# CarminLiu/ORB_SLAM2_aruco

Hardware: AMD Instinct MI355X
Metric: frames/s (ORB+ArUco extract+match, 640x480 mono) (higher is better)
Workload: dtype u8

## Files before the change

### orb_slam2_aruco_amd/csrc/match_kernels.hip

```cpp
#include <climits>

#include "host_stage.hpp"
#include "orbfe_common.hpp"
#include "wave_dpp.hpp"

namespace orbfe {

__device__ __forceinline__ int hamming256(const uint4& a0, const uint4& a1, const uint4& b0, const uint4& b1)
{
    int d = __popc(a0.x ^ b0.x);
    d += __popc(a0.y ^ b0.y);
    d += __popc(a0.z ^ b0.z);
    d += __popc(a0.w ^ b0.w);
    d += __popc(a1.x ^ b1.x);
    d += __popc(a1.y ^ b1.y);
    d += __popc(a1.z ^ b1.z);
    d += __popc(a1.w ^ b1.w);
    return d;
}

#define KNN_TILE 256

__global__ __launch_bounds__(256) void k_knn2_tiles(const uint8_t* __restrict__ Q, const int32_t* __restrict__ nq_arr,
                                                    size_t q_stride, int max_nq, const uint8_t* __restrict__ T,
                                                    const int32_t* __restrict__ nt_arr, size_t t_stride, int chunk,
                                                    int init, int32_t* __restrict__ best_idx,
                                                    int32_t* __restrict__ best_dist, int32_t* __restrict__ second_dist)
{
    __shared__ uint4 st[KNN_TILE * 2];
    const int pair = blockIdx.y, split = blockIdx.z, nsplit = gridDim.z;
    const int nq = nq_arr ? nq_arr[pair] : max_nq;
    const int nt = nt_arr[pair];
    const int q = blockIdx.x * 256 + threadIdx.x;
    if (blockIdx.x * 256 >= nq) return;
    const uint4* Qp = reinterpret_cast<const uint4*>(Q + (size_t)pair * q_stride);
    const uint4* Tp = reinterpret_cast<const uint4*>(T + (size_t)pair * t_stride);
    uint4 a0 = make_uint4(0, 0, 0, 0), a1 = a0;
    if (q < nq) { a0 = Qp[2 * q]; a1 = Qp[2 * q + 1]; }
    int best = init, second = init, idx = -1;
    const int t_begin = split * chunk, t_end = min(nt, t_begin + chunk);
    for (int t0 = t_begin; t0 < t_end; t0 += KNN_TILE) {
        const int m = min(KNN_TILE, t_end - t0);
        __syncthreads();
        for (int i = threadIdx.x; i < 2 * m; i += 256) st[i] = Tp[2 * t0 + i];
        __syncthreads();
        for (int t = 0; t < m; t++) {
            const int d = hamming256(a0, a1, st[2 * t], st[2 * t + 1]);
            if (d < best) { second = best; best = d; idx = t0 + t; }
            else if (d < second) second = d;
        }
    }
    if (q < nq) {
        const size_t o = ((size_t)pair * nsplit + split) * max_nq + q;
        best_idx[o] = idx; best_dist[o] = best; second_dist[o] = second;
    }
}

#define KM_WAVES 8
#define KM_CHUNK 128
#define KM_ROWB 272
typedef int v4i __attribute__((ext_vector_type(4)));
typedef int v16i __attribute__((ext_vector_type(16)));

__device__ __forceinline__ int med3i(int a, int b, int c) { return max(min(a, b), min(max(a, b), c)); }
__device__ __forceinline__ int spread4(uint32_t x) { return (int)(__umul24(x & 15u, 0x00204081u) & 0x01010101u); }
__device__ __forceinline__ int x255_1(int x)
{
    int t;
    asm("v_lshlrev_b32 %0, 8, %1" : "=v"(t) : "v"(x));
    return t - x;
}
__device__ __forceinline__ v4i x255(v4i p)
{
    v4i r;
    r.x = x255_1(p.x); r.y = x255_1(p.y); r.z = x255_1(p.z); r.w = x255_1(p.w);
    return r;
}
__device__ __forceinline__ v4i spread16(uint32_t bits)
{
    v4i r;
    r.x = spread4(bits); r.y = spread4(bits >> 4); r.z = spread4(bits >> 8); r.w = spread4(bits >> 12);
    return r;
}

__global__ __launch_bounds__(KM_WAVES * 64) __attribute__((amdgpu_waves_per_eu(4, 4))) void k_knn2_mfma(const uint8_t* __restrict__ Q, const int32_t* __restrict__ nq_arr,
                                                             size_t q_stride, int max_nq, const uint8_t* __restrict__ T,
                                                             const int32_t* __restrict__ nt_arr, size_t t_stride, int chunk,
                                                             int init, int32_t* __restrict__ best_idx,
                                                             int32_t* __restrict__ best_dist,
                                                             int32_t* __restrict__ second_dist)
{
    constexpr int KM_LDS = KM_CHUNK * KM_ROWB > KM_WAVES * 32 * 33 * 4 ? KM_CHUNK * KM_ROWB : KM_WAVES * 32 * 33 * 4;
    __shared__ __align__(16) unsigned char s_u[KM_LDS];
    unsigned char* s_t = s_u;
    int (*s_red)[32][33] = reinterpret_cast<int (*)[32][33]>(s_u);
    __shared__ int s_pt[KM_CHUNK];
    const int pair = blockIdx.y, tid = threadIdx.x, lane = tid & 63, wid = tid >> 6;
    const int nq = nq_arr ? nq_arr[pair] : max_nq;
    const int split = blockIdx.z, nsplit = gridDim.z;
    const int t_begin = split * chunk, nt = min(nt_arr[pair], t_begin + chunk);
    const int q0 = blockIdx.x * (KM_WAVES * 32);
    if (q0 >= nq) return;
    const uint32_t* Qp = reinterpret_cast<const uint32_t*>(Q + (size_t)pair * q_stride);
    const uint32_t* Tp = reinterpret_cast<const uint32_t*>(T + (size_t)pair * t_stride);
    const int col = lane & 31, half = lane >> 5;
    const int ie = min(init, 257);

    const int qa = q0 + 32 * wid + col;
    v4i a[8];
    {
        const uint4* qrow = reinterpret_cast<const uint4*>(Qp) + (size_t)min(qa, nq - 1) * 2;
        const uint4 d0 = qrow[0], d1 = qrow[1];
        const uint32_t w[8] = {d0.x, d0.y, d0.z, d0.w, d1.x, d1.y, d1.z, d1.w};
#pragma unroll
        for (int s2 = 0; s2 < 8; s2++) {
            const v4i p = spread16((qa < nq ? w[s2] : 0u) >> (16 * half));
            a[s2] = x255(p);
        }
    }
    int bestk[16], secondk[16];
#pragma unroll
    for (int r = 0; r < 16; r++) bestk[r] = secondk[r] = 0x7fffffff;

    const int ctr = tid >> 2, cpart = tid & 3;
    const uint2* Tp2 = reinterpret_cast<const uint2*>(Tp);
    uint2 nxt = make_uint2(0u, 0u);
    if (t_begin < nt) nxt = Tp2[(size_t)min(t_begin + ctr, nt - 1) * 4 + cpart];
    for (int t0 = t_begin; t0 < nt; t0 += KM_CHUNK) {
        const int m = min(KM_CHUNK, nt - t0);
        uint2 w = nxt;
        if (ctr >= m) w = make_uint2(0u, 0u);
        __syncthreads();
        {
            v4i* dst = reinterpret_cast<v4i*>(s_t + ctr * KM_ROWB + cpart * 64);
            dst[0] = spread16(w.x);
            dst[1] = spread16(w.x >> 16);
            dst[2] = spread16(w.y);
            dst[3] = spread16(w.y >> 16);
            int pc = __popc(w.x) + __popc(w.y);
            pc += ORBFE_DPP(0, pc, 0xb1, 0xf);
            pc += ORBFE_DPP(0, pc, 0x4e, 0xf);
            if (cpart == 0) s_pt[ctr] = pc;
        }
        if (t0 + KM_CHUNK < nt) nxt = Tp2[(size_t)min(t0 + KM_CHUNK + ctr, nt - 1) * 4 + cpart];
        __syncthreads();
#pragma unroll
        for (int tt = 0; tt < KM_CHUNK; tt += 32) {
            v16i acc = {0, 0, 0, 0, 0, 0, 0, 0, 0, 0, 0, 0, 0, 0, 0, 0};
            const unsigned char* brow = s_t + (tt + col) * KM_ROWB + 16 * half;
            v4i b[8];
#pragma unroll
            for (int s2 = 0; s2 < 8; s2++) b[s2] = *reinterpret_cast<const v4i*>(brow + 32 * s2);
            const int pt = s_pt[tt + col];
#pragma unroll
            for (int s2 = 0; s2 < 8; s2++) acc = __builtin_amdgcn_mfma_i32_32x32x32_i8(a[s2], b[s2], acc, 0, 0, 0);
            const uint32_t cj = (tt + col < m) ? (((uint32_t)pt << 16) | (uint32_t)(t0 + tt + col)) : 0x7fffffffu;
#pragma unroll
            for (int r = 0; r < 16; r++) {
                const int key = (int)(((uint32_t)acc[r] << 17) + cj);
                secondk[r] = med3i(bestk[r], secondk[r], key);
                bestk[r] = min(bestk[r], key);
            }
        }
    }
    __syncthreads();
#pragma unroll
    for (int pass = 0; pass < 2; pass++) {
        __builtin_amdgcn_wave_barrier();
#pragma unroll
        for (int r = 0; r < 16; r++) s_red[wid][(r & 3) + 8 * (r >> 2) + 4 * half][col] = pass == 0 ? bestk[r] : secondk[r];
        __builtin_amdgcn_wave_barrier();
        int b1 = 0x7fffffff, b2 = 0x7fffffff;
#pragma unroll
        for (int c = 0; c < 16; c++) {
            const int key = s_red[wid][col][16 * half + c];
            b2 = med3i(b1, b2, key);
            b1 = min(b1, key);
        }
        const int o1 = __shfl_xor(b1, 32), o2 = __shfl_xor(b2, 32);
        const int n1 = min(b1, o1);
        const int n2 = min(max(b1, o1), min(b2, o2));
        if (pass == 0) { bestk[0] = n1; bestk[1] = n2; }
        else { secondk[0] = n1; }
    }
    if (half == 0) {
        const int qr = q0 + 32 * wid + col;
        if (qr < nq) {
            uint4 d0 = reinterpret_cast<const uint4*>(Qp)[(size_t)qr * 2], d1 = reinterpret_cast<const uint4*>(Qp)[(size_t)qr * 2 + 1];
            const int pq = __popc(d0.x) + __popc(d0.y) + __popc(d0.z) + __popc(d0.w) + __popc(d1.x) + __popc(d1.y) + __popc(d1.z) + __popc(d1.w);
            const int kb = bestk[0], ks = min(bestk[1], secondk[0]);
            int bd = (kb >> 16) + pq, sd = (ks >> 16) + pq, bi = kb & 0xffff;
            if (bd >= ie) { bd = init; bi = -1; }
            if (sd >= ie) sd = init;
            const size_t o = ((size_t)pair * nsplit + split) * max_nq + qr;
            best_idx[o] = bi; best_dist[o] = bd; second_dist[o] = sd;
        }
    }
}

__global__ void k_knn2_merge(const int32_t* __restrict__ pidx, const int32_t* __restrict__ pbest,
                             const int32_t* __restrict__ psecond, int nsplit, int max_nq,
                             const int32_t* __restrict__ nq_arr, int32_t* __restrict__ best_idx,
                             int32_t* __restrict__ best_dist, int32_t* __restrict__ second_dist)
{
    const int pair = blockIdx.y;
    const int q = blockIdx.x * blockDim.x + threadIdx.x;
    const int nq = nq_arr ? nq_arr[pair] : max_nq;
    if (q >= nq) return;
    int best = INT_MAX, second = INT_MAX, idx = -1;
    for (int s = 0; s < nsplit; s++) {
        const size_t o = ((size_t)pair * nsplit + s) * max_nq + q;
        const int b = pbest[o], sc = psecond[o], i = pidx[o];
        if (s == 0) { best = b; second = sc; idx = i; continue; }
        if (b < best) { second = min(best, sc); best = b; idx = i; }
        else second = min(second, b);
    }
    const size_t o = (size_t)pair * max_nq + q;
    best_idx[o] = idx; best_dist[o] = best; second_dist[o] = second;
}

#define GRID_COLS 64
#define GRID_ROWS 48


#define SFI_MAXL0 1024
struct SfiGrid {
    int32_t* nl0;
    int32_t* nq;
    uint32_t* sorted;
    float2* xy;
    float* ang;
    uint4* desc;
    uint16_t* query;
    float2* qxy;
    int32_t* cursor;
};
#define SFI_GRID_THREADS 256
#define SFI_CURSOR_PAD 64
#define SFI_ROWS_BX 64
#define SFI_POOL_LDS 6144
#define SFI_ROW_BITS 11

__global__ __launch_bounds__(SFI_GRID_THREADS) void k_sfi_grid(const orbfe_keypoint* __restrict__ kps, const uint8_t* __restrict__ desc,
                                                               const int32_t* __restrict__ nkp, int capacity, int nframes, float4 bnd,
                                                               SfiGrid G, int32_t* __restrict__ overflow)
{
    __shared__ __align__(16) uint32_t s_key[SFI_MAXL0 + 4];
    __shared__ int s_nl0;
    const int f = blockIdx.x, tid = threadIdx.x, lane = tid & 63, wid = tid >> 6;
    const orbfe_keypoint* k = kps + (size_t)f * capacity;
    const uint8_t* d = desc + (size_t)f * capacity * 32;
    const int n = nkp[f];
    const float mnMinX = bnd.x, mnMinY = bnd.y;
    const float invW = __fdiv_rn((float)GRID_COLS, bnd.z - bnd.x);
    const float invH = __fdiv_rn((float)GRID_ROWS, bnd.w - bnd.y);
    if (tid == 0) { s_nl0 = 0; if (f < nframes - 1) G.cursor[(size_t)f * SFI_CURSOR_PAD] = 0; }
    __syncthreads();
    for (int i = tid; i < n; i += SFI_GRID_THREADS) {
        const orbfe_keypoint kp = k[i];
        if (kp.octave != 0) continue;
        const int px = (int)roundf(__fmul_rn(kp.x - mnMinX, invW));
        const int py = (int)roundf(__fmul_rn(kp.y - mnMinY, invH));
        if (px >= 0 && px < GRID_COLS && py >= 0 && py < GRID_ROWS) {
            const int e = atomicAdd(&s_nl0, 1);
            if (e < SFI_MAXL0) s_key[e] = ((uint32_t)(px * GRID_ROWS + py) << 16) | (uint32_t)i;
        }
    }
    if (wid == 0) {
        int nq = 0;
        uint16_t* qo = G.query + (size_t)f * SFI_MAXL0;
        float2* qp = G.qxy + (size_t)f * SFI_MAXL0;
        for (int i0 = 0; i0 < n; i0 += 64) {
            const int i = i0 + lane;
            orbfe_keypoint kp;
            kp.octave = 1;
            if (i < n) kp = k[i];
            const bool isq = i < n && kp.octave <= 0;
            const unsigned long long m = __ballot(isq);
            const int pos = nq + __builtin_amdgcn_mbcnt_hi((unsigned)(m >> 32), __builtin_amdgcn_mbcnt_lo((unsigned)m, 0));
            if (isq && pos < SFI_MAXL0) { qo[pos] = (uint16_t)i; qp[pos] = make_float2(kp.x, kp.y); }
            nq += __popcll(m);
        }
        if (lane == 0) {
            if (nq > SFI_MAXL0) { atomicMax(overflow, nq); nq = SFI_MAXL0; }
            G.nq[f] = nq;
        }
    }
    __syncthreads();
    int nl0 = s_nl0;
    if (nl0 > SFI_MAXL0) { if (tid == 0) atomicMax(overflow, nl0); nl0 = SFI_MAXL0; }
    if (tid == 0) G.nl0[f] = nl0;
    if (tid < 4) s_key[nl0 + tid] = 0xffffffffu;
    __syncthreads();
    const uint4* k4 = reinterpret_cast<const uint4*>(s_key);
    for (int e = tid; e < nl0; e += SFI_GRID_THREADS) {
        const uint32_t key = s_key[e];
        int r = 0;
        for (int j = 0; j < (nl0 + 3) / 4; j++) {
            const uint4 v = k4[j];
            r += (v.x < key) + (v.y < key) + (v.z < key) + (v.w < key);
        }
        const int i2 = key & 0xffff;
        const orbfe_keypoint kp = k[i2];
        const size_t o = (size_t)f * SFI_MAXL0 + r;
        G.sorted[o] = key;
        G.xy[o] = make_float2(kp.x, kp.y);
        G.ang[o] = kp.angle;
        G.desc[2 * o] = reinterpret_cast<const uint4*>(d)[2 * i2];
        G.desc[2 * o + 1] = reinterpret_cast<const uint4*>(d)[2 * i2 + 1];
    }
}

struct SfiWindow { float x, y, r; int minx, maxx, miny, maxy; };
__device__ __forceinline__ int sfi_chunks4(const SfiGrid& G, size_t g2, int nl0, int c0, int lane, const SfiWindow& W, const uint4& a0,
                                           const uint4& a1, int base, int* keys)
{
    uint32_t cell[4];
    float2 xy[4];
#pragma unroll
    for (int k = 0; k < 4; k++) {
        const int j = (c0 + k) * 64 + lane;
        cell[k] = 0xffffffffu; xy[k] = make_float2(0.f, 0.f);
        if (j < nl0) { cell[k] = G.sorted[g2 + j] >> 16; xy[k] = G.xy[g2 + j]; }
    }
    bool ok[4];
    uint4 b0[4], b1[4];
#pragma unroll
    for (int k = 0; k < 4; k++) {
        const int cx = (int)(cell[k] / GRID_ROWS), cy = (int)(cell[k] - (uint32_t)cx * GRID_ROWS);
        ok[k] = cell[k] != 0xffffffffu && cx >= W.minx && cx <= W.maxx && cy >= W.miny && cy <= W.maxy && fabsf(xy[k].x - W.x) < W.r &&
                fabsf(xy[k].y - W.y) < W.r;
        if (ok[k]) { const size_t o = 2 * (g2 + (size_t)((c0 + k) * 64 + lane)); b0[k] = G.desc[o]; b1[k] = G.desc[o + 1]; }
    }
    int n = 0;
#pragma unroll
    for (int k = 0; k < 4; k++) {
        const unsigned long long m = __ballot(ok[k]);
        keys[k] = 0x7fffffff;
        if (ok[k]) {
            const int pos = base + n + __builtin_amdgcn_mbcnt_hi((unsigned)(m >> 32), __builtin_amdgcn_mbcnt_lo((unsigned)m, 0));
            const int dd = hamming256(a0, a1, b0[k], b1[k]);
            keys[k] = (min(dd, 255) << 20) | (pos << 10) | ((c0 + k) * 64 + lane);
        }
        n += (int)__popcll(m);
// ... 681 lines not shown
    int nlevels, strict_max, level_below, level_above;
    float log_scale, th;
    int use_T2;
    float T2[12];
    int frame_variant;
};

__global__ __launch_bounds__(256) void k_project_map_points(const float* __restrict__ p3Dw, const uint8_t* __restrict__ valid,
                                                            const float* __restrict__ min_dist, const float* __restrict__ max_dist,
                                                            const float* __restrict__ normal, int n, ProjectParams P,
                                                            SbpQuery* __restrict__ queries)
{
    const int i = blockIdx.x * 256 + threadIdx.x;
    if (i >= n) return;
    SbpQuery Q{0.0f, 0.0f, -1.0f, 0, 0};
    if (!valid || valid[i]) {
        const float X = p3Dw[3 * i], Y = p3Dw[3 * i + 1], Z = p3Dw[3 * i + 2];
        float xc = __fadd_rn(__fadd_rn(__fadd_rn(__fmul_rn(P.T[0], X), __fmul_rn(P.T[1], Y)), __fmul_rn(P.T[2], Z)), P.T[3]);
        float yc = __fadd_rn(__fadd_rn(__fadd_rn(__fmul_rn(P.T[4], X), __fmul_rn(P.T[5], Y)), __fmul_rn(P.T[6], Z)), P.T[7]);
        float zc = __fadd_rn(__fadd_rn(__fadd_rn(__fmul_rn(P.T[8], X), __fmul_rn(P.T[9], Y)), __fmul_rn(P.T[10], Z)), P.T[11]);
        if (P.use_T2) {
            const float a = xc, b = yc, c = zc;
            xc = __fadd_rn(__fadd_rn(__fadd_rn(__fmul_rn(P.T2[0], a), __fmul_rn(P.T2[1], b)), __fmul_rn(P.T2[2], c)), P.T2[3]);
            yc = __fadd_rn(__fadd_rn(__fadd_rn(__fmul_rn(P.T2[4], a), __fmul_rn(P.T2[5], b)), __fmul_rn(P.T2[6], c)), P.T2[7]);
            zc = __fadd_rn(__fadd_rn(__fadd_rn(__fmul_rn(P.T2[8], a), __fmul_rn(P.T2[9], b)), __fmul_rn(P.T2[10], c)), P.T2[11]);
        }
        float u = 0.0f, v = 0.0f;
        bool inside = false;
        if (P.frame_variant) {
            const float invzc = (float)(1.0 / (double)zc);
            u = __fadd_rn(__fmul_rn(__fmul_rn(P.K[0], xc), invzc), P.K[2]);
            v = __fadd_rn(__fmul_rn(__fmul_rn(P.K[1], yc), invzc), P.K[3]);
            inside = u >= P.bnd[0] && u <= P.bnd[2] && v >= P.bnd[1] && v <= P.bnd[3];
        } else if (!(zc < 0.0f)) {
            const float invz = __fdiv_rn(1.0f, zc);
            u = __fadd_rn(__fmul_rn(P.K[0], __fmul_rn(xc, invz)), P.K[2]);
            v = __fadd_rn(__fmul_rn(P.K[1], __fmul_rn(yc, invz)), P.K[3]);
            inside = P.strict_max ? (u >= P.bnd[0] && u < P.bnd[2] && v >= P.bnd[1] && v < P.bnd[3])
                                  : (u >= P.bnd[0] && u <= P.bnd[2] && v >= P.bnd[1] && v <= P.bnd[3]);
        }
        if (inside) {
            const float px = P.use_T2 ? xc : X - P.Ow[0], py = P.use_T2 ? yc : Y - P.Ow[1], pz = P.use_T2 ? zc : Z - P.Ow[2];
            const float dist3D = (float)sqrt((double)px * px + (double)py * py + (double)pz * pz);
            const float mfMax = max_dist[i];
            bool ok = !(dist3D < __fmul_rn(0.8f, min_dist[i]) || dist3D > __fmul_rn(1.2f, mfMax));
            if (ok && normal) {
                const double dot = (double)px * normal[3 * i] + (double)py * normal[3 * i + 1] + (double)pz * normal[3 * i + 2];
                ok = !(dot < 0.5 * (double)dist3D);
            }
            if (ok) {
                const float ratio = __fdiv_rn(mfMax, dist3D);
                int lvl = (int)ceilf(__fdiv_rn((float)log((double)ratio), P.log_scale));
                if (lvl < 0) lvl = 0;
                else if (lvl >= P.nlevels) lvl = P.nlevels - 1;
                Q = SbpQuery{u, v, __fmul_rn(P.th, P.scale[lvl]), lvl - P.level_below, lvl + P.level_above};
            }
        }
    }
    queries[i] = Q;
}

#define DD_MAXN 256
__global__ __launch_bounds__(256) void k_distinctive(const uint8_t* __restrict__ desc, const int32_t* __restrict__ offsets, int npoints,
                                                     int32_t* __restrict__ best_idx, uint8_t* __restrict__ best_desc)
{
    const int p = blockIdx.x * 4 + (threadIdx.x >> 6), lane = threadIdx.x & 63;
    if (p >= npoints) return;
    const int o0 = offsets[p], N = min(offsets[p + 1] - o0, DD_MAXN);
    if (N <= 0) {
        if (lane == 0) best_idx[p] = -1;
        return;
    }
    const uint4* D = reinterpret_cast<const uint4*>(desc) + (size_t)o0 * 2;
    uint32_t w[4][8];
#pragma unroll
    for (int c = 0; c < 4; c++) {
        const int j = lane + 64 * c;
        uint4 a = make_uint4(0, 0, 0, 0), b = a;
        if (j < N) { a = D[2 * j]; b = D[2 * j + 1]; }
        w[c][0] = a.x; w[c][1] = a.y; w[c][2] = a.z; w[c][3] = a.w; w[c][4] = b.x; w[c][5] = b.y; w[c][6] = b.z; w[c][7] = b.w;
    }
    const int k = (int)(0.5 * (double)(N - 1));
    int best_median = 0x7fffffff, best = 0;
    for (int i = 0; i < N; i++) {
        uint32_t r[8];
        const int src_lane = i & 63, src_c = i >> 6;
#pragma unroll
        for (int q = 0; q < 8; q++) {
            const uint32_t v = src_c == 0 ? w[0][q] : src_c == 1 ? w[1][q] : src_c == 2 ? w[2][q] : w[3][q];
            r[q] = (uint32_t)__builtin_amdgcn_readlane((int)v, src_lane);
        }
        int d[4];
#pragma unroll
        for (int c = 0; c < 4; c++) {
            int s_ = 0;
#pragma unroll
            for (int q = 0; q < 8; q++) s_ += __popc(w[c][q] ^ r[q]);
            d[c] = s_;
        }
        int lo = 0, hi = 256;
        while (lo < hi) {
            const int mid = (lo + hi) >> 1;
            int cnt = 0;
#pragma unroll
            for (int c = 0; c < 4; c++) cnt += __popcll(__ballot(lane + 64 * c < N && d[c] <= mid));
            if (cnt >= k + 1) hi = mid; else lo = mid + 1;
        }
        if (lo < best_median) { best_median = lo; best = i; }
    }
    if (lane == 0) best_idx[p] = best;
    if (best_desc && lane < 8) reinterpret_cast<uint32_t*>(best_desc)[(size_t)p * 8 + lane] = reinterpret_cast<const uint32_t*>(D)[(size_t)best * 8 + lane];
}

struct MatchWorkspace {
    DevBuf pidx, pbest, psecond, csr_cnt, csr_idx, csr_dist, scratch;
    DevBuf sbp_batch_overflow;
    DevBuf sfi_overflow;
    DevBuf q, obest;
    int csr_per_pair = 0;
    int sbp_stride = 0;
};
static thread_local ThreadWorkspaces<MatchWorkspace> tl_ws;
static MatchWorkspace& ws(hipStream_t s) { return tl_ws.get(s); }
static thread_local ThreadWorkspaces<HostStage> tl_stage;
HostStage& match_host_stage() { return tl_stage.get(); }
static int ensure_sticky_flag(DevBuf& b)
{
    if (b.p) return ORBFE_OK;
    int rc = b.ensure(16);
    if (rc) return rc;
    ORBFE_HIP(hipMemset(b.p, 0, 16));
    return ORBFE_OK;
}

static int g_knn2_path = 0;
#ifdef ORBFE_ABLATION
int g_orb_skip = 0, g_aruco_skip = 0;
#endif

static int knn2_launch(const uint8_t* d_Q, const int32_t* d_nq, size_t q_stride, int max_nq, const uint8_t* d_T,
                       const int32_t* d_nt, size_t t_stride, int max_nt, int npairs, int init, int32_t* d_best_idx,
                       int32_t* d_best_dist, int32_t* d_second_dist, hipStream_t s)
{
    const bool mfma_ok = max_nt <= 65535 && init > 0;
    const bool use_mfma = mfma_ok && g_knn2_path != 1;
    const int qtiles = (max_nq + 255) / 256;
    int nsplit = 1, chunk;
    const long long wgs = (long long)qtiles * npairs;
    if (use_mfma) {
        const int max_split = (max_nt + KM_CHUNK - 1) / KM_CHUNK;
        if (wgs < 512) nsplit = (int)std::max<long long>(1, std::min<long long>(512 / wgs, max_split));
        chunk = (max_nt + nsplit - 1) / nsplit;
        chunk = std::max(KM_CHUNK, (chunk + KM_CHUNK - 1) / KM_CHUNK * KM_CHUNK);
    } else {
        if (wgs < 1024) {
            nsplit = (int)std::min<long long>((1024 + wgs - 1) / wgs, (max_nt + KNN_TILE - 1) / KNN_TILE);
            if (nsplit < 1) nsplit = 1;
        }
        chunk = (max_nt + nsplit - 1) / nsplit;
        chunk = std::max(KNN_TILE, (chunk + KNN_TILE - 1) / KNN_TILE * KNN_TILE);
    }
    nsplit = std::max(1, (max_nt + chunk - 1) / chunk);
    const dim3 mgrid((max_nq + KM_WAVES * 32 - 1) / (KM_WAVES * 32), npairs, nsplit);
    if (nsplit == 1) {
        if (use_mfma)
            hipLaunchKernelGGL(k_knn2_mfma, mgrid, dim3(KM_WAVES * 64), 0, s, d_Q, d_nq, q_stride, max_nq, d_T, d_nt, t_stride, chunk, init,
                               d_best_idx, d_best_dist, d_second_dist);
        else
            hipLaunchKernelGGL(k_knn2_tiles, dim3(qtiles, npairs, 1), dim3(256), 0, s, d_Q, d_nq, q_stride, max_nq, d_T,
                               d_nt, t_stride, chunk, init, d_best_idx, d_best_dist, d_second_dist);
    } else {
        MatchWorkspace& w = ws(s);
        const size_t nb = (size_t)npairs * nsplit * max_nq * 4;
        int rc;
        if ((rc = w.pidx.ensure(nb)) || (rc = w.pbest.ensure(nb)) || (rc = w.psecond.ensure(nb))) return rc;
        if (use_mfma)
            hipLaunchKernelGGL(k_knn2_mfma, mgrid, dim3(KM_WAVES * 64), 0, s, d_Q, d_nq, q_stride, max_nq, d_T, d_nt, t_stride, chunk, init,
                               w.pidx.as<int32_t>(), w.pbest.as<int32_t>(), w.psecond.as<int32_t>());
        else
            hipLaunchKernelGGL(k_knn2_tiles, dim3(qtiles, npairs, nsplit), dim3(256), 0, s, d_Q, d_nq, q_stride, max_nq,
                               d_T, d_nt, t_stride, chunk, init, w.pidx.as<int32_t>(), w.pbest.as<int32_t>(),
                               w.psecond.as<int32_t>());
        hipLaunchKernelGGL(k_knn2_merge, dim3(qtiles, npairs), dim3(256), 0, s, w.pidx.as<int32_t>(),
                           w.pbest.as<int32_t>(), w.psecond.as<int32_t>(), nsplit, max_nq, d_nq, d_best_idx,
                           d_best_dist, d_second_dist);
    }
    ORBFE_HIP(hipGetLastError());
    return ORBFE_OK;
}

static float4 frame_bounds(int cols, int rows, const float* bounds)
{
    return bounds ? make_float4(bounds[0], bounds[1], bounds[2], bounds[3]) : make_float4(0.f, 0.f, (float)cols, (float)rows);
}

static int sfi_launch(const orbfe_keypoint* d_kps, const uint8_t* d_desc, const int32_t* d_n, int capacity, int npairs,
                      float4 bnd, int window, float nnratio, int check_ori, const float* d_prev_in,
                      float* d_prev_out, int32_t* d_m12, int32_t* d_nm, hipStream_t s, MatchWorkspace& w)
{
    if (capacity > 65535) return fail(ORBFE_ERR_INVALID, "capacity above 65535 keypoints per frame is unsupported");
    const int pool_cap = std::max((w.csr_per_pair + 3) / 4 * 4, 16384);
    w.csr_per_pair = pool_cap;
    const int nframes = npairs + 1;
    const size_t F = (size_t)nframes * SFI_MAXL0;
    int rc;
    if ((rc = w.csr_cnt.ensure((size_t)nframes * (2 + SFI_CURSOR_PAD) * 4 + 64)) || (rc = w.csr_idx.ensure(F * (4 + 8 + 4 + 32 + 8 + 2) + 256)) ||
        (rc = w.csr_dist.ensure((size_t)npairs * pool_cap * 4 + 512 )) || (rc = w.scratch.ensure((size_t)npairs * SFI_MAXL0 * 4)))
        return rc;
    if (!w.sfi_overflow.p) {
        if ((rc = w.sfi_overflow.ensure(16))) return rc;
        ORBFE_HIP(hipMemset(w.sfi_overflow.p, 0, 16));
    }
    SfiGrid G;
    G.nl0 = w.csr_cnt.as<int32_t>();
    G.nq = G.nl0 + nframes;
    G.cursor = G.nq + nframes;
    uint8_t* b = w.csr_idx.as<uint8_t>();
    G.desc = reinterpret_cast<uint4*>(b); b += F * 32;
    G.xy = reinterpret_cast<float2*>(b); b += F * 8;
    G.sorted = reinterpret_cast<uint32_t*>(b); b += F * 4;
    G.qxy = reinterpret_cast<float2*>(b); b += F * 8;
    G.ang = reinterpret_cast<float*>(b); b += F * 4;
    G.query = reinterpret_cast<uint16_t*>(b);
    int32_t* ovf = w.sfi_overflow.as<int32_t>();
    hipLaunchKernelGGL(k_sfi_grid, dim3(nframes), dim3(SFI_GRID_THREADS), 0, s, d_kps, d_desc, d_n, capacity, nframes, bnd, G, ovf);
    hipLaunchKernelGGL(k_sfi_rows, dim3(SFI_ROWS_BX, npairs), dim3(SFI_ROWS_WAVES * 64), 0, s, d_kps, d_desc, capacity, bnd, (float)window, d_prev_in, G,
                       w.csr_dist.as<uint32_t>(), pool_cap, w.scratch.as<uint32_t>(), ovf);
    hipLaunchKernelGGL(k_sfi_accept, dim3(npairs), dim3(64), 0, s, d_kps, d_n, capacity, nnratio, check_ori, d_prev_in, d_prev_out, d_m12,
                       d_nm, G, w.csr_dist.as<uint32_t>(), pool_cap, w.scratch.as<uint32_t>());
    ORBFE_HIP(hipGetLastError());
    return ORBFE_OK;
}

static int sfi_take_flags(MatchWorkspace& w, const int32_t* f, hipStream_t s, int32_t* need)
{
    if (f[0] || f[1]) ORBFE_HIP(hipMemsetAsync(w.sfi_overflow.p, 0, 8, s));
    if (f[1] > w.csr_per_pair) w.csr_per_pair = (f[1] + 1023) / 1024 * 1024;
    *need = f[0] > SFI_MAXL0 ? f[0] : f[1];
    if (f[0] > SFI_MAXL0) return fail(ORBFE_ERR_CAPACITY, "%d level-0 keypoints in a frame exceed the supported %d", f[0], SFI_MAXL0);
    return ORBFE_OK;
}

static void sbp_grow_stride(MatchWorkspace& w, int overflow)
{
    if (overflow > w.sbp_stride) w.sbp_stride = (overflow + 63) / 64 * 64;
}

static int sbp_launch(MatchWorkspace& w, SbpBatch B, int nframes, float4 bnd, int mode, int th_high, float nnratio, float factor,
                      int check_ori, hipStream_t s)
{
    if (B.capacity > 65535) return fail(ORBFE_ERR_INVALID, "more than 65535 keypoints per frame are unsupported");
    int ncap = 64;
    while (ncap < B.capacity) ncap <<= 1;
    const size_t lds = (size_t)ncap * (4 + 8 + 1 + 1) + (SBP_CELLS + 2) * 2 + 64;
    if (lds > 150 * 1024) return fail(ORBFE_ERR_CAPACITY, "%d keypoints do not fit the grid kernel's LDS", B.capacity);
    w.sbp_stride = std::max(w.sbp_stride, 128);
    const size_t NQ = (size_t)nframes * B.qcapacity;
    int rc;
    if ((rc = w.csr_idx.ensure(NQ * w.sbp_stride * 2)) || (rc = w.csr_dist.ensure(NQ * w.sbp_stride)) || (rc = w.csr_cnt.ensure(NQ * 4)) ||
        (rc = ensure_dyn_lds(reinterpret_cast<const void*>(&k_search_by_projection_batch), lds)))
        return rc;
    B.row_rank = w.csr_idx.as<uint16_t>(); B.row_dist = w.csr_dist.as<uint8_t>(); B.row_cnt = w.csr_cnt.as<int32_t>(); B.row_stride = w.sbp_stride;
    hipLaunchKernelGGL(k_search_by_projection_batch, dim3(nframes), dim3(SBP_THREADS), lds, s, B, ncap, bnd, mode, th_high, nnratio, factor,
                       check_ori);
    ORBFE_HIP(hipGetLastError());
    return ORBFE_OK;
}

struct SbpHostCall {
    const orbfe_keypoint* kps; const uint8_t* desc; int n; float4 bnd;
    const uint8_t* taken;
    int nq; const uint8_t* qdesc; const uint8_t* q_observed; const float* q_angle;
    const orbfe_window_query* window;
    const float* x3Dw; const uint8_t* valid;
    const orbfe_keypoint* kps_last; const float* Tcw; const float* K4; const float* scale; int nlevels; float th;
    const ProjectParams* P; const float* min_dist; const float* max_dist; const float* normal;
    int mode, th_high; float nnratio, factor; int check_ori;
    double chi2; const float* inv_sigma2;
    int32_t *best_idx, *best_dist, *best_level, *second_dist, *second_level, *match, *match_cur, *nmatches;
    uint8_t* taken_out;
};

static int sbp_host_run(const SbpHostCall& c)
{
    HostStage& w = match_host_stage();
    const size_t n = (size_t)c.n, nq = (size_t)c.nq, kb = sizeof(orbfe_keypoint);
    IoLayout l;
    const size_t s_kps = l.take(n * kb), s_desc = l.take(n * 32), s_q = l.take(nq * sizeof(SbpQuery)), s_qdesc = l.take(nq * 32);
    const size_t s_obs = l.take(nq), s_angle = l.take(nq * 4), s_x3 = l.take(nq * 12), s_valid = l.take(nq);
    const size_t s_last = l.take(c.kps_last ? nq * kb : 0), s_cam = l.take(c.kps_last ? (12 + 16) * 4 : 0);
    const size_t s_min = l.take(c.P ? nq * 4 : 0), s_max = l.take(c.P ? nq * 4 : 0), s_nrm = l.take(c.P ? nq * 12 : 0);
    l.inout();
    const size_t s_taken = l.take(n), s_cnt = l.take(8);
    l.outputs();
    const size_t s_cur = l.take(n * 4), s_out = l.take(nq * 4 * 7);
    int rc = w.begin(l);
    if (rc) return rc;
    const hipStream_t s = w.stream;
    MatchWorkspace& m = ws(s);
    int32_t* o = w.dev<int32_t>(s_out);
    SbpBatch B{};
    B.kps = w.dev<const orbfe_keypoint>(s_kps); B.desc = w.dev<const uint8_t>(s_desc); B.capacity = c.n;
    B.queries = w.dev<const SbpQuery>(s_q); B.qdesc = w.dev<const uint8_t>(s_qdesc); B.qcapacity = c.nq;
    B.taken = c.taken ? w.dev<uint8_t>(s_taken) : nullptr; B.q_observed = c.q_observed ? w.dev<const uint8_t>(s_obs) : nullptr;
    B.q_angle = c.q_angle || c.kps_last ? w.dev<const float>(s_angle) : nullptr;
    if (c.best_idx) { B.best_idx = o; B.best_dist = o + nq; B.best_level = o + 2 * nq; B.second_dist = o + 3 * nq; B.second_level = o + 4 * nq; }
// ... 636 lines not shown
```

Baseline: 260,900.

## Fold target popcount and index packing into an extra MFMA K-step

Re-encodes the query and target bit-expansions so that a single i8 MFMA accumulation, plus one extra 32x32x16 MFMA over a per-row tail (column bias and local index bytes), yields a packed key of Hamming-related distance and local index directly. This removes the per-chunk popcount/DPP reduction, the s_pt shared array, and the per-element shift-and-add key construction in the inner loop. It also splits the loop into full chunks and a templated tail tile so bounds checks disappear on the common path. The chunk is capped at 4096 targets so the 12-bit local index fits, which can raise the split count for large target sets.

```diff
diff --git a/orb_slam2_aruco_amd/csrc/match_kernels.hip b/orb_slam2_aruco_amd/csrc/match_kernels.hip
--- a/orb_slam2_aruco_amd/csrc/match_kernels.hip
+++ b/orb_slam2_aruco_amd/csrc/match_kernels.hip
@@ -59,28 +59,46 @@
 #define KM_WAVES 8
 #define KM_CHUNK 128
 #define KM_ROWB 272
+#define KM_MAXT 4096
 typedef int v4i __attribute__((ext_vector_type(4)));
 typedef int v16i __attribute__((ext_vector_type(16)));
 
 __device__ __forceinline__ int med3i(int a, int b, int c) { return max(min(a, b), min(max(a, b), c)); }
-__device__ __forceinline__ int spread4(uint32_t x) { return (int)(__umul24(x & 15u, 0x00204081u) & 0x01010101u); }
-__device__ __forceinline__ int x255_1(int x)
-{
-    int t;
-    asm("v_lshlrev_b32 %0, 8, %1" : "=v"(t) : "v"(x));
-    return t - x;
-}
-__device__ __forceinline__ v4i x255(v4i p)
-{
-    v4i r;
-    r.x = x255_1(p.x); r.y = x255_1(p.y); r.z = x255_1(p.z); r.w = x255_1(p.w);
-    return r;
-}
+__device__ __forceinline__ int spread4(uint32_t x) { return (int)(((x & 15u) * 0x08102040u) & 0x40404040u); }
 __device__ __forceinline__ v4i spread16(uint32_t bits)
 {
     v4i r;
     r.x = spread4(bits); r.y = spread4(bits >> 4); r.z = spread4(bits >> 8); r.w = spread4(bits >> 12);
     return r;
+}
+__device__ __forceinline__ v4i query_bytes(v4i p)
+{
+    v4i r;
+    r.x = (p.x << 1) | 0x40404040; r.y = (p.y << 1) | 0x40404040; r.z = (p.z << 1) | 0x40404040; r.w = (p.w << 1) | 0x40404040;
+    return r;
+}
+
+template <bool TAIL>
+__device__ __forceinline__ void km_tile(const unsigned char* s_t, int tt, int col, int half, const v4i (&a)[8], long a9, int m,
+                                        int (&bestk)[16], int (&secondk)[16])
+{
+    v16i acc = {0, 0, 0, 0, 0, 0, 0, 0, 0, 0, 0, 0, 0, 0, 0, 0};
+    const unsigned char* brow = s_t + (tt + col) * KM_ROWB;
+    v4i b[8];
+#pragma unroll
+    for (int s2 = 0; s2 < 8; s2++) b[s2] = *reinterpret_cast<const v4i*>(brow + 16 * half + 32 * s2);
+    const long b9 = *reinterpret_cast<const long*>(brow + 256);
+#pragma unroll
+    for (int s2 = 0; s2 < 8; s2++) acc = __builtin_amdgcn_mfma_i32_32x32x32_i8(a[s2], b[s2], acc, 0, 0, 0);
+    acc = __builtin_amdgcn_mfma_i32_32x32x16_i8(a9, b9, acc, 0, 0, 0);
+    const bool live = !TAIL || tt + col < m;
+#pragma unroll
+    for (int r = 0; r < 16; r++) {
+        const int key = live ? acc[r] : 0x7fffffff;
+        secondk[r] = med3i(bestk[r], secondk[r], key);
+        bestk[r] = min(bestk[r], key);
+    }
+    __builtin_amdgcn_sched_barrier(0);
 }
 
 __global__ __launch_bounds__(KM_WAVES * 64) __attribute__((amdgpu_waves_per_eu(4, 4))) void k_knn2_mfma(const uint8_t* __restrict__ Q, const int32_t* __restrict__ nq_arr,
@@ -94,7 +112,6 @@
     __shared__ __align__(16) unsigned char s_u[KM_LDS];
     unsigned char* s_t = s_u;
     int (*s_red)[32][33] = reinterpret_cast<int (*)[32][33]>(s_u);
-    __shared__ int s_pt[KM_CHUNK];
     const int pair = blockIdx.y, tid = threadIdx.x, lane = tid & 63, wid = tid >> 6;
     const int nq = nq_arr ? nq_arr[pair] : max_nq;
     const int split = blockIdx.z, nsplit = gridDim.z;
@@ -113,11 +130,9 @@
         const uint4 d0 = qrow[0], d1 = qrow[1];
         const uint32_t w[8] = {d0.x, d0.y, d0.z, d0.w, d1.x, d1.y, d1.z, d1.w};
 #pragma unroll
-        for (int s2 = 0; s2 < 8; s2++) {
-            const v4i p = spread16((qa < nq ? w[s2] : 0u) >> (16 * half));
-            a[s2] = x255(p);
-        }
-    }
+        for (int s2 = 0; s2 < 8; s2++) a[s2] = query_bytes(spread16((qa < nq ? w[s2] : 0u) >> (16 * half)));
+    }
+    const long a9 = half == 0 ? 0x0140L : 0L;
     int bestk[16], secondk[16];
 #pragma unroll
     for (int r = 0; r < 16; r++) bestk[r] = secondk[r] = 0x7fffffff;
@@ -126,8 +141,7 @@
     const uint2* Tp2 = reinterpret_cast<const uint2*>(Tp);
     uint2 nxt = make_uint2(0u, 0u);
     if (t_begin < nt) nxt = Tp2[(size_t)min(t_begin + ctr, nt - 1) * 4 + cpart];
-    for (int t0 = t_begin; t0 < nt; t0 += KM_CHUNK) {
-        const int m = min(KM_CHUNK, nt - t0);
+    auto stage = [&](int t0, int m) {
         uint2 w = nxt;
         if (ctr >= m) w = make_uint2(0u, 0u);
         __syncthreads();
@@ -137,31 +151,26 @@
             dst[1] = spread16(w.x >> 16);
             dst[2] = spread16(w.y);
             dst[3] = spread16(w.y >> 16);
-            int pc = __popc(w.x) + __popc(w.y);
-            pc += ORBFE_DPP(0, pc, 0xb1, 0xf);
-            pc += ORBFE_DPP(0, pc, 0x4e, 0xf);
-            if (cpart == 0) s_pt[ctr] = pc;
+            if (cpart == 0) {
+                const uint32_t j = (uint32_t)(t0 - t_begin + ctr);
+                *reinterpret_cast<uint2*>(s_t + ctr * KM_ROWB + 256) = make_uint2((j >> 6) | ((j & 63u) << 8), 0u);
+            }
         }
         if (t0 + KM_CHUNK < nt) nxt = Tp2[(size_t)min(t0 + KM_CHUNK + ctr, nt - 1) * 4 + cpart];
         __syncthreads();
-#pragma unroll
-        for (int tt = 0; tt < KM_CHUNK; tt += 32) {
-            v16i acc = {0, 0, 0, 0, 0, 0, 0, 0, 0, 0, 0, 0, 0, 0, 0, 0};
-            const unsigned char* brow = s_t + (tt + col) * KM_ROWB + 16 * half;
-            v4i b[8];
-#pragma unroll
-            for (int s2 = 0; s2 < 8; s2++) b[s2] = *reinterpret_cast<const v4i*>(brow + 32 * s2);
-            const int pt = s_pt[tt + col];
-#pragma unroll
-            for (int s2 = 0; s2 < 8; s2++) acc = __builtin_amdgcn_mfma_i32_32x32x32_i8(a[s2], b[s2], acc, 0, 0, 0);
-            const uint32_t cj = (tt + col < m) ? (((uint32_t)pt << 16) | (uint32_t)(t0 + tt + col)) : 0x7fffffffu;
-#pragma unroll
-            for (int r = 0; r < 16; r++) {
-                const int key = (int)(((uint32_t)acc[r] << 17) + cj);
-                secondk[r] = med3i(bestk[r], secondk[r], key);
-                bestk[r] = min(bestk[r], key);
-            }
-        }
+    };
+    int t0 = t_begin;
+    for (; t0 + KM_CHUNK <= nt; t0 += KM_CHUNK) {
+        stage(t0, KM_CHUNK);
+#pragma unroll
+        for (int tt = 0; tt < KM_CHUNK; tt += 32) km_tile<false>(s_t, tt, col, half, a, a9, KM_CHUNK, bestk, secondk);
+    }
+    if (t0 < nt) {
+        const int m = nt - t0;
+        stage(t0, m);
+        int tt = 0;
+        for (; tt + 32 <= m; tt += 32) km_tile<false>(s_t, tt, col, half, a, a9, m, bestk, secondk);
+        if (tt < m) km_tile<true>(s_t, tt, col, half, a, a9, m, bestk, secondk);
     }
     __syncthreads();
 #pragma unroll
@@ -189,7 +198,7 @@
             uint4 d0 = reinterpret_cast<const uint4*>(Qp)[(size_t)qr * 2], d1 = reinterpret_cast<const uint4*>(Qp)[(size_t)qr * 2 + 1];
             const int pq = __popc(d0.x) + __popc(d0.y) + __popc(d0.z) + __popc(d0.w) + __popc(d1.x) + __popc(d1.y) + __popc(d1.z) + __popc(d1.w);
             const int kb = bestk[0], ks = min(bestk[1], secondk[0]);
-            int bd = (kb >> 16) + pq, sd = (ks >> 16) + pq, bi = kb & 0xffff;
+            int bd = (kb >> 12) + pq, sd = (ks >> 12) + pq, bi = (kb & (KM_MAXT - 1)) + t_begin;
             if (bd >= ie) { bd = init; bi = -1; }
             if (sd >= ie) sd = init;
             const size_t o = ((size_t)pair * nsplit + split) * max_nq + qr;
@@ -1177,6 +1186,7 @@
         if (wgs < 512) nsplit = (int)std::max<long long>(1, std::min<long long>(512 / wgs, max_split));
         chunk = (max_nt + nsplit - 1) / nsplit;
         chunk = std::max(KM_CHUNK, (chunk + KM_CHUNK - 1) / KM_CHUNK * KM_CHUNK);
+        chunk = std::min(chunk, KM_MAXT);
     } else {
         if (wgs < 1024) {
             nsplit = (int)std::min<long long>((1024 + wgs - 1) / wgs, (max_nt + KNN_TILE - 1) / KNN_TILE);
```

Result: faster. 265,100 (median of 6 runs) (+1.6%).
